# yekaizhou/duet

Measured on AMD Instinct MI355X. Metric: SV support-read marks clustered+phased /sec; bit-exact phased_sv.vcf vs ref, higher is better.
Workload: dtype u32/u64 integer + f64 threshold compares; 1 GPU; BASELINE configs[1]: synthetic 1 contig, 1001116 SV marks / 100000 candidates / 159991 tagged reads, resident in HBM; step = ef_classify + ef_finalize_own, two launches (phasing, E/F; ef_seed_sort 0: ; marks_per_gpu=1001116, candidates_per_gpu=100000, reads_per_gpu=159991, parallelism=contig-sharded x1, svlen_thres=50, suppread_thres=2, device_preheat_steps=2900

## Files before the change

### duet_amd/csrc/duet_ef.hip

```cpp

#include <hip/hip_runtime.h>
#include <hip/hip_ext.h>
#include <stdint.h>
#include <stdio.h>
#include <stdlib.h>
#include <string.h>
#include <string>
#include <vector>

#include "duet_ef.h"
#include "duet_internal.h"

#pragma clang fp contract(off)

namespace {

#ifdef DUET_STAMPS
#define STAMP(k, i) do { if (threadIdx.x == 0 && p.stamps) p.stamps[((size_t)(k) * 65536 + blockIdx.x) * 8 + (i)] = wall_clock64(); } while (0)
#else
#define STAMP(k, i) do { } while (0)
#endif

#include "duet_seeds.hip.h"

// ... 361 lines not shown
                v.t1 = st.TA1; v.t2 = st.TA2;
                bool need_fp = false;
                int pred = (p.dbg & DUET_DBG_EF_FP_DECIDE) ? 0 : decide01_int((int)n_ps, v, deg, svread, refread, need_fp);
                need_fp = need_fp || (p.dbg & DUET_DBG_EF_FP_DECIDE) != 0;
                if (need_fp) pred = decide((int)n_ps, v, deg, svread, refread);
                code = (uint8_t)pred;
                ps_out = st.ps_a == kEmpty ? 0u : st.ps_a;
                if (n_ps == 0 || (st.a1 == 0 && st.a2 == 0)) code |= kNeedNearest;
            }
        }
        p.out_pred[c] = code;
        p.out_ps[c] = ps_out;
    }
    return want_seed ? st.seed() : kEmpty;
}

__device__ __forceinline__ void seeds_tile(const Params &p, TileShared &sh, uint32_t tile, uint32_t tid, uint32_t c,
                                           uint32_t is_start, bool owner = true)
{
    const uint32_t seed = owner ? sh.seed[tid] : kEmpty;
    const bool want_seed = seed != kEmpty;
    const uint32_t lane = tid & 63u, wave = tid >> 6;
    const unsigned long long wmask = __ballot(want_seed);
    const unsigned long long smask = __ballot(is_start != 0);
    const unsigned long long upto = lane == 63 ? ~0ull : ((1ull << (lane + 1)) - 1ull);
    if (lane == 0 && owner) {
        if (wmask) {
            const uint32_t li = 63u - (uint32_t)__clzll(wmask);
            sh.wlast[wave] = sh.seed[wave * 64 + li];
            sh.wclean[wave] = (li == 63 || (smask >> (li + 1)) == 0) ? 1u : 0u;
        } else {
            sh.wlast[wave] = kEmpty;
            sh.wclean[wave] = 0;
        }
    }
    __syncthreads();
    bool keep = want_seed;
    if (want_seed) {
        const unsigned long long lower = wmask & (upto >> 1);
        if (lower) {
            const uint32_t pl = 63u - (uint32_t)__clzll(lower);
            const unsigned long long between = smask & upto & ~((1ull << (pl + 1)) - 1ull);
            keep = !(between == 0 && sh.seed[wave * 64 + pl] == seed);
        } else if (wave > 0) {
            keep = !((smask & upto) == 0 && sh.wclean[wave - 1] && sh.wlast[wave - 1] == seed);
        }
    }
    const unsigned long long mask = __ballot(keep);
    if (lane == 0 && owner) sh.wcnt[wave] = (uint32_t)__popcll(mask);
    __syncthreads();
    uint32_t before = 0, total = 0;
#pragma unroll
    for (uint32_t w = 0; w < kCandPerBlock / 64; ++w) {
        before += w < wave ? sh.wcnt[w] : 0u;
        total += sh.wcnt[w];
    }
    if (keep) {
        const uint32_t at = before + (uint32_t)__popcll(mask & (upto >> 1));
        const uint64_t e = ((uint64_t)c << 32) | seed;
        if (at < 7) p.blk_rec[(size_t)tile * 8 + 1 + at] = e;
        if (at >= 3) p.seed_ent[(size_t)tile * kCandPerBlock + at] = e;
    }
    if (tid == 0) p.blk_rec[(size_t)tile * 8] = total;
}

__device__ __forceinline__ void issue_fence()
{
    asm volatile("" ::: "memory");
    __builtin_amdgcn_sched_barrier(0);
}

template <int NT = kCandPerBlock, int IT>
__device__ __forceinline__ void stage_load_marks(const uint32_t *__restrict__ mark_read, uint4 (&r)[IT], uint32_t cs, uint32_t m_end,
                                                 uint32_t tid)
{
#pragma unroll
    for (int it = 0; it < IT; ++it) {
        const uint32_t m = cs + 4u * (tid + it * NT);
        r[it] = *reinterpret_cast<const uint4 *>(mark_read + (m < m_end ? m : cs));
    }
    issue_fence();
}

template <int IT>
__device__ __forceinline__ void stage_gather(const uint64_t *__restrict__ read_tag, const uint64_t *__restrict__ untagged, uint32_t n_reads,
                                             uint64_t (&t)[4 * IT], const uint4 (&r)[IT])
{
#pragma unroll
    for (int it = 0; it < IT; ++it) {
        uint32_t idx[4] = {r[it].x, r[it].y, r[it].z, r[it].w};
        asm volatile("" : "+v"(idx[0]), "+v"(idx[1]), "+v"(idx[2]), "+v"(idx[3])::"memory");
#pragma unroll
        for (int j = 0; j < 4; ++j) {
            const uint64_t *a = idx[j] < n_reads ? read_tag + idx[j] : untagged;
            t[4 * it + j] = *a;
        }
        issue_fence();
    }
}

template <int NT = kCandPerBlock, int IT4>
__device__ __forceinline__ void stage_store(uint64_t *s_tag, const uint64_t (&t)[IT4], uint32_t tid)
{
#pragma unroll
    for (int it = 0; it < IT4 / 4; ++it) {
        const uint32_t i = 4u * (tid + it * NT);
#pragma unroll
        for (int j = 0; j < 4; ++j) s_tag[i + j] = t[4 * it + j];
    }
}

template <bool VEC, bool DYN = false>
__global__ __launch_bounds__(kCandPerBlock, 6) void ef_classify(const Params p)
{
    __shared__ uint64_t s_tag[kChunk];
    __shared__ uint32_t s_span[2];
    __shared__ TileShared sh;

    const uint32_t tid = threadIdx.x;
    STAMP(0, 0);
    const uint32_t C = p.C, n_reads = p.n_reads, svlen_thres = p.svlen_thres, suppread_thres = p.suppread_thres;
    const uint32_t heavy_t = min(p.heavy_t, 255u);
    const uint32_t *__restrict__ const cand_off = p.cand_off, *__restrict__ const mark_read = p.mark_read;
    const uint64_t *__restrict__ const read_tag = p.read_tag, *__restrict__ const untagged = p.untagged;
    const uint32_t *__restrict__ const cand_svlen = p.cand_svlen, *__restrict__ const cand_svread = p.cand_svread;
    const uint32_t *__restrict__ const cand_refread = p.cand_refread;
    const uint8_t *__restrict__ const cand_gt_ok = p.cand_gt_ok, *__restrict__ const ctg_start = p.ctg_start;
    asm volatile("" ::"s"(C), "s"(n_reads), "s"(svlen_thres), "s"(suppread_thres), "s"(heavy_t), "s"(cand_off), "s"(mark_read),
                 "s"(read_tag), "s"(untagged), "s"(cand_svlen), "s"(cand_svread), "s"(cand_refread), "s"(cand_gt_ok), "s"(ctg_start));
    asm volatile("" ::"s"(p.dbg), "s"(p.out_pred), "s"(p.out_ps), "s"(p.blk_rec), "s"(p.seed_ent), "s"(p.c2rec), "s"(p.status),
                 "s"(p.c2_fixed), "s"(p.c2_cap));
    uint32_t n_cands = C;
    for (uint32_t tile = blockIdx.x;; tile += gridDim.x) {
        const uint32_t c0 = tile * kCandPerBlock, c = c0 + tid;
        const uint32_t ic = min(c, C - 1u);
        const uint32_t o0_ld = cand_off[min(c, C)], o1_ld = cand_off[min(c + 1u, C)];
        const uint32_t svlen_ld = cand_svlen[ic], svread_ld = cand_svread[ic], refread_ld = cand_refread[ic], gt_ld = cand_gt_ok[ic];
        uint32_t start_ld = 0, cc0_ld = 0, cc1_ld = 0, mb_ld = 0, me_ld = 0;
        if constexpr (DYN) {
            if (p.cand_contig) {
                cc0_ld = p.cand_contig[ic];
                cc1_ld = p.cand_contig[max(ic, 1u) - 1u];
            }
        } else {
            start_ld = ctg_start[ic];
            mb_ld = cand_off[c0];
            me_ld = cand_off[min(c0 + (uint32_t)kCandPerBlock, C)];
        }
        if constexpr (DYN) {
            uint32_t zero = 0;
            asm volatile("" : "+s"(zero));
            n_cands = p.dyn_c[zero];
            if (c0 >= n_cands) break;
        }
        const uint32_t nc = min((uint32_t)kCandPerBlock, n_cands - c0);
        asm volatile("" ::"v"(o0_ld), "v"(o1_ld), "v"(svlen_ld), "v"(svread_ld), "v"(refread_ld), "v"(gt_ld), "v"(start_ld), "v"(cc0_ld),
                     "v"(cc1_ld));
        if (tid == 0) sh.c2n = 0;
        const bool live = tid < nc;
        const uint32_t svlen = svlen_ld, svread = svread_ld, refread = refread_ld, gt_ok = gt_ld;
        uint32_t is_start = 0;
        if constexpr (DYN) {
            if (p.cand_contig) {
                is_start = (live && (c == 0 || cc0_ld != cc1_ld)) ? 1u : 0u;
            } else if (live) {
                uint32_t k = p.blk_ctg[tile];
                while (c >= p.ctg_off[k + 1]) ++k;
                is_start = c == p.ctg_off[k] ? 1u : 0u;
            }
        } else {
            is_start = live ? start_ld : 0u;
        }
        const bool kept = live && svlen >= svlen_thres && svread >= suppread_thres && gt_ok != 0;
        const bool divzero = kept && ((uint64_t)svread + (uint64_t)refread == 0);
        uint32_t m_begin, m_end;
        if constexpr (DYN) {
            if (tid == 0) s_span[0] = o0_ld;
            if (tid == nc - 1u) s_span[1] = o1_ld;
            lds_barrier();
            m_begin = s_span[0]; m_end = s_span[1];
        } else {
            m_begin = mb_ld; m_end = me_ld;
        }
        m_begin = (uint32_t)__builtin_amdgcn_readfirstlane((int)m_begin);
        m_end = (uint32_t)__builtin_amdgcn_readfirstlane((int)m_end);
        STAMP(0, 1);

        const uint32_t j = tid;
        const bool active = kept && !divzero;
        const uint32_t my_b = live ? o0_ld : 0, my_e = live ? o1_ld : 0;
        CandState st;

        const uint32_t base = VEC ? (m_begin & ~3u) : m_begin;
        for (uint32_t cs = base; cs < m_end; cs += kChunk) {
            if (VEC) {
                uint4 r[kStageIt];
                uint64_t t[4 * kStageIt];
                stage_load_marks(mark_read, r, cs, m_end, tid);
                stage_gather(read_tag, untagged, n_reads, t, r);
                stage_store(s_tag, t, tid);
            } else {
                for (uint32_t i = tid; i < kChunk && cs + i < m_end; i += kCandPerBlock) {
                    const uint32_t r = mark_read[cs + i];
                    s_tag[i] = r < n_reads ? read_tag[r] : kUntagged;
                }
            }
            __syncthreads();
            STAMP(0, 2);
            uint32_t lo = max(my_b, cs);
            const uint32_t hi = min(my_e, cs + (uint32_t)kChunk);
            if (!kept) lo = hi;
            const bool heavy = lo < hi && my_e - my_b > heavy_t;
            unsigned long long hm = __ballot(heavy);
            consume_range(st, s_tag, heavy ? hi : lo, hi, cs);
            while (hm) {
                const uint32_t h = (uint32_t)__builtin_amdgcn_readfirstlane((int)((uint32_t)__ffsll((long long)hm) - 1u));
                hm &= hm - 1ull;
                const uint32_t lo_h = (uint32_t)__builtin_amdgcn_readlane((int)lo, h), hi_h = (uint32_t)__builtin_amdgcn_readlane((int)hi, h);
                consume_heavy(st, s_tag, lo_h, hi_h, cs, tid & 63u, h);
            }
            STAMP(0, 3);
            __syncthreads();
        }
        STAMP(0, 4);
        uint32_t c2_rank;
        const uint32_t seed = decide_store(p, sh, tile, live, c0 + j, active, divzero, st, my_e - my_b, svread, refread, c2_rank);
        sh.seed[j] = seed;
        __syncthreads();
        if (sh.c2n > kC2Quota) {
            if (tid == 0) sh.c2base = atomicAdd(&p.status[1], sh.c2n - kC2Quota);
            __syncthreads();
            if (live && c2_rank != kEmpty && c2_rank >= kC2Quota) {
                const uint32_t at = sh.c2base + (c2_rank - kC2Quota);
                if (at < p.c2_cap - p.c2_fixed) {
                    store_summary(p, p.c2_fixed + at, st);
                    p.out_pred[c0 + j] = kClass2;
                    p.out_ps[c0 + j] = p.c2_fixed + at;
                }
            }
        }
        seeds_tile(p, sh, tile, tid, c0 + tid, is_start);
        STAMP(0, 6);
        if (!DYN) break;
        __syncthreads();
    }
}

constexpr int kSplit = 2;
constexpr int kSplitThreads = kSplit * kCandPerBlock;
constexpr int kSplitChunk = kChunk;
constexpr int kSplitStagers = 384;
constexpr int kSplitStageIt = kSplitChunk / (kSplitStagers * 4);
constexpr uint32_t kSplitMaxTiles = 512;
static_assert(kSplit == 2 || kSplit == 4, "the parts are halves, or halves of halves");
static_assert(kSplitStageIt >= 1 && kSplitStageIt * kSplitStagers * 4 == kSplitChunk, "a pass is whole 16-byte loads");
static_assert(kSplitStagers % 64 == 0 && kSplitStagers <= kSplitThreads, "whole wavefronts stage");

__device__ __forceinline__ void split_bounds(uint32_t b, uint32_t e, uint32_t part, uint32_t &lo, uint32_t &hi)
{
    lo = b; hi = e;
#pragma unroll
    for (uint32_t bit = kSplit >> 1; bit != 0; bit >>= 1) {
        const uint32_t mid = lo + (hi - lo + 1u) / 2u;
        if (part & bit) lo = mid; else hi = mid;
    }
}

__device__ __forceinline__ void fold(CandState &l, const CandState &r)
{
    l.multi = l.multi || r.multi || (l.first_ps != kEmpty && r.first_ps != kEmpty && l.first_ps != r.first_ps);
    l.first_ps = min(l.first_ps, r.first_ps);
    l.nv += r.nv;
    auto take = [&](uint32_t ps, uint32_t n, uint32_t h1, uint32_t h2, uint32_t t1, uint32_t t2) {
        const bool is = ps != kEmpty;
        const bool to_a = is && (l.ps_a == kEmpty || l.ps_a == ps);
        const bool to_b = is && !to_a && (l.ps_b == kEmpty || l.ps_b == ps);
        l.ps_a = to_a ? ps : l.ps_a;
        l.a1 += to_a ? h1 : 0u; l.a2 += to_a ? h2 : 0u;
        l.TA1 += to_a ? t1 : 0u; l.TA2 += to_a ? t2 : 0u;
        l.ps_b = to_b ? ps : l.ps_b;
        l.n_b += to_b ? n : 0u;
        l.b1 += to_b ? h1 : 0u; l.b2 += to_b ? h2 : 0u;
        l.tb1 += to_b ? t1 : 0u; l.tb2 += to_b ? t2 : 0u;
        l.more = l.more || (is && !to_a && !to_b);
    };
    take(r.ps_a, r.nv - r.n_b, r.a1, r.a2, (uint32_t)r.TA1, (uint32_t)r.TA2);
    take(r.ps_b, r.n_b, r.b1, r.b2, r.tb1, r.tb2);
    l.more = l.more || r.more;
    l.n_a = l.more ? (l.ps_a != kEmpty ? 1u : 0u) : l.nv - l.n_b;
}

__device__ __forceinline__ void hand_store(uint4 (*s_hand)[(kSplit - 1) * kCandPerBlock], uint32_t slot, const CandState &st)
{
    s_hand[0][slot] = make_uint4(st.first_ps, st.ps_a, st.ps_b, st.nv | st.n_b << 8 | (st.multi ? 1u << 16 : 0u) | (st.more ? 1u << 17 : 0u));
    s_hand[1][slot] = make_uint4(st.a1 << 24 | (uint32_t)st.TA1, st.a2 << 24 | (uint32_t)st.TA2, st.b1 << 24 | st.tb1, st.b2 << 24 | st.tb2);
}

__device__ __forceinline__ CandState hand_load(const uint4 (*s_hand)[(kSplit - 1) * kCandPerBlock], uint32_t slot)
{
    const uint4 x = s_hand[0][slot], y = s_hand[1][slot];
    CandState st;
    st.first_ps = x.x; st.ps_a = x.y; st.ps_b = x.z;
    st.nv = x.w & 0xFFu; st.n_b = (x.w >> 8) & 0xFFu; st.multi = (x.w >> 16 & 1u) != 0; st.more = (x.w >> 17 & 1u) != 0;
    st.a1 = y.x >> 24; st.a2 = y.y >> 24; st.b1 = y.z >> 24; st.b2 = y.w >> 24;
    st.TA1 = y.x & 0xFFFFFFu; st.TA2 = y.y & 0xFFFFFFu; st.tb1 = y.z & 0xFFFFFFu; st.tb2 = y.w & 0xFFFFFFu;
    return st;
}

template <bool VEC>
__global__ __launch_bounds__(kSplitThreads, 6) void ef_classify_split(const Params p)
{
    __shared__ uint64_t s_tag[kSplitChunk];
    __shared__ uint4 s_hand[2][(kSplit - 1) * kCandPerBlock];
    __shared__ TileShared sh;

    const uint32_t tid = threadIdx.x, j = tid % kCandPerBlock, part = tid / kCandPerBlock;
    const bool owner = part == 0;
    STAMP(0, 0);
    const uint32_t C = p.C, n_reads = p.n_reads, svlen_thres = p.svlen_thres, suppread_thres = p.suppread_thres;
    const uint32_t heavy_t = min(p.heavy_t, 255u);
    const uint32_t *__restrict__ const cand_off = p.cand_off, *__restrict__ const mark_read = p.mark_read;
    const uint64_t *__restrict__ const read_tag = p.read_tag, *__restrict__ const untagged = p.untagged;
    const uint32_t *__restrict__ const cand_svlen = p.cand_svlen, *__restrict__ const cand_svread = p.cand_svread;
    const uint32_t *__restrict__ const cand_refread = p.cand_refread;
    const uint8_t *__restrict__ const cand_gt_ok = p.cand_gt_ok, *__restrict__ const ctg_start = p.ctg_start;
    asm volatile("" ::"s"(C), "s"(n_reads), "s"(svlen_thres), "s"(suppread_thres), "s"(heavy_t), "s"(cand_off), "s"(mark_read),
                 "s"(read_tag), "s"(untagged), "s"(cand_svlen), "s"(cand_svread), "s"(cand_refread), "s"(cand_gt_ok), "s"(ctg_start));
    asm volatile("" ::"s"(p.dbg), "s"(p.out_pred), "s"(p.out_ps), "s"(p.blk_rec), "s"(p.seed_ent), "s"(p.c2rec), "s"(p.status),
                 "s"(p.c2_fixed), "s"(p.c2_cap));
    const uint32_t tile = blockIdx.x, c0 = tile * kCandPerBlock, c = c0 + j;
    const uint32_t ic = min(c, C - 1u);
    const uint32_t o0_ld = cand_off[min(c, C)], o1_ld = cand_off[min(c + 1u, C)];
    const uint32_t svlen_ld = cand_svlen[ic], svread_ld = cand_svread[ic], refread_ld = cand_refread[ic], gt_ld = cand_gt_ok[ic];
    const uint32_t start_ld = ctg_start[ic];
    const uint32_t mb_ld = cand_off[c0], me_ld = cand_off[min(c0 + (uint32_t)kCandPerBlock, C)];
    const uint32_t nc = min((uint32_t)kCandPerBlock, C - c0);
    asm volatile("" ::"v"(o0_ld), "v"(o1_ld), "v"(svlen_ld), "v"(svread_ld), "v"(refread_ld), "v"(gt_ld), "v"(start_ld));
    if (tid == 0) sh.c2n = 0;
    const bool live = j < nc;
    const uint32_t svlen = svlen_ld, svread = svread_ld, refread = refread_ld, gt_ok = gt_ld;
    const uint32_t is_start = (owner && live) ? start_ld : 0u;
    const bool kept = live && svlen >= svlen_thres && svread >= suppread_thres && gt_ok != 0;
    const bool divzero = kept && ((uint64_t)svread + (uint64_t)refread == 0);
    const uint32_t m_begin = (uint32_t)__builtin_amdgcn_readfirstlane((int)mb_ld);
    const uint32_t m_end = (uint32_t)__builtin_amdgcn_readfirstlane((int)me_ld);
    STAMP(0, 1);

    const bool active = kept && !divzero;
    const uint32_t my_b = live ? o0_ld : 0, my_e = live ? o1_ld : 0;
    const bool heavy_c = my_e - my_b > heavy_t;
    uint32_t w_b, w_e;
    split_bounds(my_b, my_e, part, w_b, w_e);
    if (heavy_c) { w_b = my_b; w_e = owner ? my_e : my_b; }
    if (!kept) w_e = w_b;
    CandState st;

    const uint32_t base = VEC ? (m_begin & ~3u) : m_begin;
    for (uint32_t cs = base; cs < m_end; cs += kSplitChunk) {
        if (VEC) {
            if (tid < kSplitStagers) {
                uint4 r[kSplitStageIt];
                uint64_t t[4 * kSplitStageIt];
                stage_load_marks<kSplitStagers>(mark_read, r, cs, m_end, tid);
                stage_gather(read_tag, untagged, n_reads, t, r);
                stage_store<kSplitStagers>(s_tag, t, tid);
            }
        } else {
            for (uint32_t i = tid; i < kSplitChunk && cs + i < m_end; i += kSplitThreads) {
                const uint32_t r = mark_read[cs + i];
                s_tag[i] = r < n_reads ? read_tag[r] : kUntagged;
            }
        }
        __syncthreads();
        STAMP(0, 2);
        const uint32_t lo = max(w_b, cs), hi = min(w_e, cs + (uint32_t)kSplitChunk);
        const bool heavy = heavy_c && lo < hi;
        unsigned long long hm = __ballot(heavy);
        consume_range(st, s_tag, heavy ? hi : lo, hi, cs);
        while (hm) {
            const uint32_t h = (uint32_t)__builtin_amdgcn_readfirstlane((int)((uint32_t)__ffsll((long long)hm) - 1u));
            hm &= hm - 1ull;
            const uint32_t lo_h = (uint32_t)__builtin_amdgcn_readlane((int)lo, h), hi_h = (uint32_t)__builtin_amdgcn_readlane((int)hi, h);
            consume_heavy(st, s_tag, lo_h, hi_h, cs, tid & 63u, h);
        }
        STAMP(0, 3);
        if (!owner && cs + (uint32_t)kSplitChunk >= m_end) hand_store(s_hand, tid - kCandPerBlock, st);
        __syncthreads();
    }
    STAMP(0, 4);
    uint32_t c2_rank = kEmpty;
    if (owner) {
        if (base < m_end) {
#pragma unroll
            for (int k = 1; k < kSplit; ++k) fold(st, hand_load(s_hand, (k - 1) * kCandPerBlock + j));
        }
        sh.seed[j] = decide_store(p, sh, tile, live, c, active, divzero, st, my_e - my_b, svread, refread, c2_rank);
    }
    __syncthreads();
    if (sh.c2n > kC2Quota) {
        if (tid == 0) sh.c2base = atomicAdd(&p.status[1], sh.c2n - kC2Quota);
        __syncthreads();
        if (owner && live && c2_rank != kEmpty && c2_rank >= kC2Quota) {
            const uint32_t at = sh.c2base + (c2_rank - kC2Quota);
            if (at < p.c2_cap - p.c2_fixed) {
                store_summary(p, p.c2_fixed + at, st);
                p.out_pred[c] = kClass2;
                p.out_ps[c] = p.c2_fixed + at;
            }
        }
    }
    seeds_tile(p, sh, tile, tid, c, is_start, owner);
    STAMP(0, 6);
}


__device__ void bitonic_sort(uint32_t *a, uint32_t n, uint32_t tid, uint32_t nthreads)
{
    uint32_t lN = 0;
    while ((1u << lN) < n) ++lN;
    const uint32_t pairs = (1u << lN) >> 1;
    for (uint32_t lk = 1; lk <= lN; ++lk) {
        const uint32_t k = 1u << lk, half = k >> 1;
        for (uint32_t i = tid; i < pairs; i += nthreads) {
            const uint32_t base = (i >> (lk - 1)) << lk, off = i & (half - 1);
            const uint32_t x = base + off, y = base + (k - 1 - off);
            if (y < n) {
                const uint32_t ax = a[x], ay = a[y];
                if (ax > ay) { a[x] = ay; a[y] = ax; }
            }
        }
        __syncthreads();
        for (int lj = (int)lk - 2; lj >= 0; --lj) {
            const uint32_t j = 1u << lj;
            for (uint32_t i = tid; i < pairs; i += nthreads) {
                const uint32_t x = ((i >> lj) << (lj + 1)) + (i & (j - 1)), y = x + j;
                if (y < n) {
                    const uint32_t ax = a[x], ay = a[y];
                    if (ax > ay) { a[x] = ay; a[y] = ax; }
                }
            }
            __syncthreads();
        }
    }
}

__device__ bool oddeven_rounds(uint32_t *a, uint32_t n, uint32_t tid, uint32_t nthreads, uint32_t *s_flag, int max_rounds)
{
    for (int r = 0; r < max_rounds; ++r) {
        if (tid == 0) *s_flag = 0;
        __syncthreads();
        for (int par = 0; par < 2; ++par) {
            for (uint32_t i = 2 * tid + par; i + 1 < n; i += 2 * nthreads) {
                const uint32_t x = a[i], y = a[i + 1];
                if (x > y) { a[i] = y; a[i + 1] = x; *s_flag = 1; }
            }
            __syncthreads();
        }
        if (*s_flag == 0) return true;
        __syncthreads();
    }
    return false;
}

__device__ uint32_t block_exscan(uint32_t v, uint32_t tid, uint32_t *s_part , uint32_t nthreads,
                                 uint32_t *total)
{
    const uint32_t lane = tid & 63u, wave = tid >> 6;
    uint32_t x = v;
#pragma unroll
    for (int d = 1; d < 64; d <<= 1) {
// ... 812 lines not shown
                                                 uint32_t me_, const uint32_t *s_tab, Vote *vo, uint32_t *pso)
{
    auto each = [&](auto f) {
        for (uint32_t m0 = mb; m0 < me_; m0 += 8) {
            uint32_t r[8];
            uint64_t t[8];
#pragma unroll
            for (int j = 0; j < 8; ++j) r[j] = tagged_index(n_reads, mark_read[m0 + j < me_ ? m0 + j : mb]);
#pragma unroll
            for (int j = 0; j < 8; ++j) t[j] = read_tag[r[j] == kEmpty ? 0u : r[j]];
#pragma unroll
            for (int j = 0; j < 8; ++j)
                if (m0 + j < me_) f(r[j] == kEmpty ? kUntagged : t[j]);
        }
    };
    auto member = [&](uint32_t key) -> bool {
        uint32_t h = (key * 2654435761u) >> (32u - 11u);
        for (;;) {
            const uint32_t v = s_tab[h];
            if (v == key) return true;
            if (v == kEmpty) return false;
            h = (h + 1u) & (kOwnTab - 1u);
        }
    };
    Vote v = {0, 0, 0, 0, 0, 0};
    uint32_t ps = 0, best = 0, done_ps = kEmpty;
    each([&](uint64_t t) {
        if (t != kUntagged && tag_pc(t) <= kPcMax) ++v.allhap;
    });
    each([&](uint64_t t) {
        if (t == kUntagged || tag_pc(t) > kPcMax) return;
        const uint32_t g = tag_ps(t);
        if (g == done_ps || (g == ps && best)) return;
        if (!member(g)) return;
        uint32_t n = 0, n1 = 0, n2 = 0;
        uint64_t s1 = 0, s2 = 0;
        each([&](uint64_t u) {
            if (u == kUntagged || tag_pc(u) > kPcMax || tag_ps(u) != g) return;
            ++n;
            const uint32_t hap = tag_hap(u), pc = tag_pc(u);
            n1 += hap == 1 ? 1u : 0u; s1 += hap == 1 ? pc : 0u;
            n2 += hap == 2 ? 1u : 0u; s2 += hap == 2 ? pc : 0u;
        });
        done_ps = g;
        if (n > best) {
            best = n; ps = g;
            v.hap1 = n1; v.hap2 = n2; v.t1 = s1; v.t2 = s2;
            v.hap0 = v.allhap - n1 - n2;
        }
    });
    *vo = v;
    *pso = ps;
}

__device__ __forceinline__ bool own_probe(uint32_t *s_tab, uint32_t key, uint32_t h)
{
    for (uint32_t probes = 0; probes < kOwnTab; ++probes) {
        const uint32_t old = atomicCAS(&s_tab[h], kEmpty, key);
        if (old == kEmpty) return true;
        if (old == key) return false;
        h = (h + 1u) & (kOwnTab - 1u);
    }
    return false;
}

constexpr uint32_t kOwnWin = 64;

template <uint32_t T>
__device__ __forceinline__ void finalize_own_tiles(const Params &p)
{
    constexpr uint32_t NT = 256u * T, NW = 4u * T;
    static_assert(kOwnTab % NT == 0 && NT <= 1024u, "the clear and own_sort_set deal the table out evenly");
    __shared__ uint32_t s_tab[kOwnTab];
    __shared__ uint32_t s_key[kOwnKeys];
    __shared__ uint32_t s_one[kOwnKeys];
    __shared__ uint32_t s_win[kOwnWin];
    __shared__ uint32_t s_mm[NW][2];
    __shared__ uint32_t s_red[NW][3];
    __shared__ uint32_t s_part[NW];
    __shared__ uint32_t s_nwin;
    __shared__ __align__(8) uint32_t s_c2[T * kC2Quota * kC2Words];
    const uint32_t tid = threadIdx.x, lane = tid & 63u, wave = tid >> 6;
    STAMP(2, 0);
    if (blockIdx.x == 0 && tid == 0) p.status[1] = 0;
    const uint32_t n_cands = p.C;
    const uint32_t nK = p.n_small;
    auto coff = [&](uint32_t kk) -> uint32_t { return p.ctg_small[kk]; };
    const uint32_t tile = blockIdx.x * T;
    const uint32_t c0 = blockIdx.x * NT, c = c0 + tid;
    const bool live = c < n_cands;
    const uint32_t cl = live ? c : n_cands - 1u;
    const uint32_t last = min(c0 + (NT - 1u), n_cands - 1);
    const uint32_t keys_cap = (p.dbg & DUET_DBG_EF_OWN_SMALLTAB) ? 8u : kOwnKeys;
    const uint32_t win_cap = (p.dbg & DUET_DBG_EF_OWN_SMALLTAB) ? 2u : kOwnWin;
    const TileRecs recs{reinterpret_cast<const ulonglong4 *>(p.blk_rec)};
    constexpr uint32_t kPre = 2;
    static_assert(kPre == 2, "the overflow loop selects between rec[0] and rec[1]");
    ulonglong4 rec[kPre], ext[kPre];
    auto load_recs = [&](uint32_t b_lo, uint32_t b_hi) {
#pragma unroll
        for (uint32_t i = 0; i < kPre; ++i) {
            const uint32_t b = min(b_lo + tid + NT * i, b_hi);
            rec[i] = recs[b];
            ext[i] = recs.second(b);
        }
    };
    const uint32_t code_ld = p.out_pred[cl], ps_ld = p.out_ps[cl], pos_ld = p.cand_pos[cl];
    const uint32_t o0_ld = p.cand_off[cl], o1_ld = p.cand_off[cl + 1u];
    const uint32_t sv_ld = p.cand_svread[cl], rf_ld = p.cand_refread[cl];
    constexpr uint32_t kPairs = T * kC2Quota * kC2Words / 2;
    static_assert(kPairs <= 2u * NT, "two pieces per thread");
    const uint2 *c2src = reinterpret_cast<const uint2 *>(p.c2rec + (size_t)tile * kC2Quota * kC2Words);
    const uint2 a0 = c2src[tid], a1 = c2src[tid + NT < kPairs ? tid + NT : tid];
    uint32_t lo = 0, hi = nK;
    while (hi - lo > 1) {
        const uint32_t mid = (lo + hi) >> 1;
        if (coff(mid) <= c0) lo = mid; else hi = mid;
    }
    uint32_t k_first = lo;
    while (k_first < nK && coff(k_first) == coff(k_first + 1)) ++k_first;
    {
        const uint32_t kf = k_first < nK ? k_first : 0u;
        load_recs(coff(kf) / kCandPerBlock, (coff(kf + 1) - 1) / kCandPerBlock);
    }
    asm volatile("" ::"v"(code_ld), "v"(ps_ld), "v"(pos_ld), "v"(o0_ld), "v"(o1_ld), "v"(sv_ld), "v"(rf_ld), "v"(a0.x), "v"(a0.y),
                 "v"(a1.x), "v"(a1.y));
    STAMP(2, 4);
    {
        uint2 *dst = reinterpret_cast<uint2 *>(s_c2);
        dst[tid] = a0;
        if (tid + NT < kPairs) dst[tid + NT] = a1;
    }
    const uint32_t code = live ? code_ld : 0u, ps_in = live ? ps_ld : 0u, c_pos = live ? pos_ld : 0u;
    const uint32_t c_o0 = live ? o0_ld : 0u, c_o1 = live ? o1_ld : 0u;
    const uint32_t c_svread = live ? sv_ld : 0u, c_refread = live ? rf_ld : 0u;
    for (uint32_t k = lo; k < nK && coff(k) <= last; ++k) {
        const uint32_t c_lo = coff(k), c_hi = coff(k + 1);
        if (c_lo == c_hi) continue;
        const uint32_t b_lo = c_lo / kCandPerBlock, b_hi = (c_hi - 1) / kCandPerBlock;
        if (k != k_first) load_recs(b_lo, b_hi);
        uint32_t t_k = threadIdx.x;
        asm volatile("" : "+v"(t_k));
        const uint32_t tid = t_k, lane = t_k & 63u, wave = t_k >> 6;
#pragma unroll
        for (uint32_t i = 0; i < kOwnTab / NT; ++i) s_tab[tid + NT * i] = kEmpty;
        if (tid == 0) s_nwin = 0;
        const bool mine = live && c >= c_lo && c < c_hi;
        const bool asks = mine && code >= 4u && !(code & kDivZero);
        {
            const uint32_t mn = wave_max_u32(asks ? ~c_pos : 0u), mx = wave_max_u32(asks ? c_pos + 1u : 0u);
            if (lane == 0) { s_mm[wave][0] = mn; s_mm[wave][1] = mx; }
        }
        lds_barrier();
        STAMP(2, 1);
        asm volatile("" ::"v"(rec[0].x), "v"(rec[1].x), "v"(rec[0].y), "v"(rec[1].y), "v"(rec[0].z), "v"(rec[1].z), "v"(rec[0].w),
                     "v"(rec[1].w), "v"(ext[0].x), "v"(ext[1].x), "v"(ext[0].y), "v"(ext[1].y), "v"(ext[0].z), "v"(ext[1].z),
                     "v"(ext[0].w), "v"(ext[1].w));
        STAMP(2, 3);
        uint32_t pmin, pmax;
        {
            uint32_t a0 = max(max(s_mm[0][0], s_mm[1][0]), max(s_mm[2][0], s_mm[3][0]));
            uint32_t a1 = max(max(s_mm[0][1], s_mm[1][1]), max(s_mm[2][1], s_mm[3][1]));
#pragma unroll
            for (uint32_t w = 4; w < NW; w += 4) {
                a0 = max(a0, max(max(s_mm[w][0], s_mm[w + 1][0]), max(s_mm[w + 2][0], s_mm[w + 3][0])));
                a1 = max(a1, max(max(s_mm[w][1], s_mm[w + 1][1]), max(s_mm[w + 2][1], s_mm[w + 3][1])));
            }
            pmin = a1 ? ~a0 : 0u;
            pmax = a1 ? a1 - 1u : 0u;
        }
        uint32_t fresh = 0, leftp = 0, rinv = 0;
        static_assert(kOwnTab == 1u << 11, "the hash takes 11 bits");
        auto slot_of = [](uint32_t key) -> uint32_t { return (key * 2654435761u) >> (32u - 11u); };
        auto count_new = [&](bool nw, uint32_t key) {
            fresh += nw ? 1u : 0u;
            leftp = max(leftp, (nw && key <= pmin) ? key + 1u : 0u);
            rinv = max(rinv, (nw && key >= pmax) ? ~key : 0u);
            if (nw && key > pmin && key < pmax) {
                const uint32_t at = atomicAdd(&s_nwin, 1u);
                if (at < kOwnWin) s_win[at] = key;
            }
        };
        auto insert = [&](uint64_t e) {
            const uint32_t cc = (uint32_t)(e >> 32), key = (uint32_t)e;
            if (cc >= c_lo && cc < c_hi) count_new(own_probe(s_tab, key, slot_of(key)), key);
        };
        uint32_t coll = 0;
        auto group = [&](const uint64_t (&e)[4], uint32_t first, uint32_t n_in, uint32_t cnt, uint32_t bit0) {
            uint32_t key[4], old[4];
            bool ok[4];
#pragma unroll
            for (uint32_t j = 0; j < 4; ++j) {
                const uint32_t cc = (uint32_t)(e[j] >> 32);
                key[j] = (uint32_t)e[j];
                ok[j] = j < n_in && first + j < cnt && cc >= c_lo && cc < c_hi;
                old[j] = kEmpty;
            }
#pragma unroll
            for (uint32_t j = 0; j < 4; ++j)
                if (ok[j]) old[j] = atomicCAS(&s_tab[slot_of(key[j])], kEmpty, key[j]);
#pragma unroll
            for (uint32_t j = 0; j < 4; ++j) {
                coll |= (ok[j] && old[j] != kEmpty && old[j] != key[j]) ? 1u << (bit0 + j) : 0u;
                count_new(ok[j] && old[j] == kEmpty, key[j]);
            }
        };
#pragma unroll
        for (uint32_t i = 0; i < kPre; ++i) {
            const uint32_t cnt = b_lo + tid + NT * i <= b_hi ? (uint32_t)rec[i].x : 0u;
            if (__any(cnt > 0u)) {
                const uint64_t e[4] = {rec[i].y, rec[i].z, rec[i].w, 0ull};
                group(e, 0u, 3u, cnt, 7u * i);
            }
            if (__any(cnt > 3u)) {
                const uint64_t e[4] = {ext[i].x, ext[i].y, ext[i].z, ext[i].w};
                group(e, 3u, 4u, cnt, 7u * i + 3u);
            }
        }
        while (coll) {
            const uint32_t j = (uint32_t)__ffs(coll) - 1u;
            coll &= coll - 1u;
            uint32_t key = 0;
#pragma unroll
            for (uint32_t i = 0; i < kPre; ++i) {
                key = j == 7u * i + 0u ? (uint32_t)rec[i].y : key;
                key = j == 7u * i + 1u ? (uint32_t)rec[i].z : key;
                key = j == 7u * i + 2u ? (uint32_t)rec[i].w : key;
                key = j == 7u * i + 3u ? (uint32_t)ext[i].x : key;
                key = j == 7u * i + 4u ? (uint32_t)ext[i].y : key;
                key = j == 7u * i + 5u ? (uint32_t)ext[i].z : key;
                key = j == 7u * i + 6u ? (uint32_t)ext[i].w : key;
            }
            count_new(own_probe(s_tab, key, (slot_of(key) + 1u) & (kOwnTab - 1u)), key);
        }
        auto overflow = [&](uint32_t b, uint32_t cnt, uint32_t from) {
            constexpr uint32_t kLong = 24;
            if (cnt > from && cnt <= kLong) {
// ... 51 lines not shown
        }
        const uint32_t n_win = s_nwin;
        const bool over = u > keys_cap;
        const bool sorted = !over && n_win > win_cap;
        if (sorted) own_sort_set<NT>(s_tab, s_key, s_one, s_part, u, tid);
        STAMP(2, 5);
        auto nearest = [&](uint32_t pos) -> uint32_t {
            if (sorted) return nearest_seed(s_one, u, pos);
            uint32_t best = 0;
            int64_t bd = -1;
            auto look = [&](uint32_t v) {
                const int64_t d = llabs((int64_t)pos - (int64_t)v);
                if (bd < 0 || d < bd || (d == bd && v > best)) { bd = d; best = v; }
            };
            if (Lp) look(Lp - 1u);
            if (Ri) look(~Ri);
            for (uint32_t i = 0; i < n_win; ++i) look(s_win[i]);
            return best;
        };
        auto member = [&](uint32_t key) -> bool {
            uint32_t h = (key * 2654435761u) >> (32u - 11u);
            for (;;) {
                const uint32_t v = s_tab[h];
                if (v == key) return true;
                if (v == kEmpty) return false;
                h = (h + 1u) & (kOwnTab - 1u);
            }
        };
        if (mine) {
            if (u == 0) {
                if (code != 0) p.out_pred[c] = 0;
                if (ps_in != 0) p.out_ps[c] = 0;
            } else if (code >= 4u) {
                if (code & kDivZero) {
                    atomicOr(&p.status[0], 1u);
                    p.out_pred[c] = 0;
                    p.out_ps[c] = 0;
                } else if (over) {
                    const OwnArgs a = {recs, p.seed_ent, p.read_tag, p.cand_pos, p.cand_off, p.cand_svread, p.cand_refread, p.mark_read, p.c2rec,
                                       p.out_ps, p.status, p.out_pred, c_lo, c_hi, p.n_reads};
                    finalize_candidate_walk(a, c, code, ps_in);
                } else if (code & kClass2Slow) {
                    Vote v;
                    uint32_t ps;
                    own_vote_from_marks(p.mark_read, p.read_tag, p.n_reads, c_o0, c_o1, s_tab, &v, &ps);
                    if (v.hap1 == 0 && v.hap2 == 0) ps = nearest(c_pos);
                    p.out_pred[c] = (uint8_t)decide(2, v, c_o1 - c_o0, c_svread, c_refread);
                    p.out_ps[c] = ps;
                } else if (code & kClass2) {
                    uint32_t w[kC2Words];
                    const uint32_t own0 = tile * kC2Quota;
                    if (ps_in >= own0 && ps_in < own0 + T * kC2Quota) {
#pragma unroll
                        for (int i = 0; i < kC2Words; ++i) w[i] = s_c2[(ps_in - own0) * kC2Words + i];
                    } else {
                        const uint32_t *rec2 = p.c2rec + (size_t)ps_in * kC2Words;
#pragma unroll
                        for (int i = 0; i < kC2Words; ++i) w[i] = rec2[i];
                    }
                    Vote v = {0, 0, 0, 0, 0, 0};
                    uint32_t ps = 0, best = 0;
                    v.allhap = w[0];
                    const uint32_t ng = w[1];
#pragma unroll
                    for (int g = 0; g < kC2Groups; ++g) {
                        if ((uint32_t)g < ng && w[2 + 6 * g + 1] > best && member(w[2 + 6 * g])) {
                            best = w[2 + 6 * g + 1];
                            ps = w[2 + 6 * g];
                            v.hap1 = w[2 + 6 * g + 2]; v.hap2 = w[2 + 6 * g + 3];
                            v.t1 = w[2 + 6 * g + 4]; v.t2 = w[2 + 6 * g + 5];
                            v.hap0 = v.allhap - v.hap1 - v.hap2;
                        }
                    }
                    if (v.hap1 == 0 && v.hap2 == 0) ps = nearest(c_pos);
                    p.out_pred[c] = (uint8_t)decide(2, v, c_o1 - c_o0, c_svread, c_refread);
                    p.out_ps[c] = ps;
                } else {
                    p.out_pred[c] = (uint8_t)(code & 3u);
                    p.out_ps[c] = nearest(c_pos);
                }
            }
        }
        STAMP(2, 6);
        __syncthreads();
    }
}

__global__ __launch_bounds__(256) void ef_finalize_own(const Params p) { finalize_own_tiles<1>(p); }

__global__ __launch_bounds__(512) void ef_finalize_own_wide(const Params p) { finalize_own_tiles<2>(p); }

__global__ void plan_mark_starts(const uint32_t *ctg_off, uint32_t K, uint8_t *ctg_start)
{
    const uint32_t k = blockIdx.x * blockDim.x + threadIdx.x;
    if (k < K && ctg_off[k] < ctg_off[k + 1]) ctg_start[ctg_off[k]] = 1;
}


}

thread_local std::string duet_g_last_error;

namespace {

inline int fail(duet_ctx *ctx, int code, const std::string &msg) { return duet_fail(ctx, code, msg); }
inline int reserve(duet_ctx *ctx, DevBuf &b, size_t bytes) { return duet_reserve(ctx, b, bytes); }

size_t c2_slots(uint32_t B, uint32_t C) { return (size_t)B * kC2Quota + (C / 8u > 256u ? C / 8u : 256u); }

struct WsWant { DevBuf *buf[6]; size_t bytes[6]; };
WsWant ws_want(duet_ctx *ctx, uint32_t K, uint32_t C, uint32_t B)
{
    const size_t small_words = (size_t)(K + 1) + K + 8 + (size_t)B + 16 + (size_t)B * 16;
    return WsWant{{&ctx->ws_small, &ctx->ws_start, &ctx->ws_ent, &ctx->ws_one, &ctx->ws_tmp, &ctx->ws_c2},
                  {small_words * 4, C, (size_t)B * kCandPerBlock * 8, ((size_t)C + K + 1) * 4, ((size_t)C + K + 1) * 4, c2_slots(B, C) * kC2Words * 4}};
}
int ws_reserve(duet_ctx *ctx, const WsWant &w, bool &grow)
{
    for (int i = 0; i < 6; ++i) grow = grow || w.bytes[i] > w.buf[i]->cap;
    if (!grow) return DUET_OK;
    HIP_TRY(ctx, hipDeviceSynchronize());
    int rc;
    for (int i = 0; i < 6; ++i)
        if ((rc = reserve(ctx, *w.buf[i], w.bytes[i]))) return rc;
    return DUET_OK;
}
void carve_small(duet_ctx *ctx, uint32_t K, uint32_t B)
{
    uint32_t *w = (uint32_t *)ctx->ws_small.ptr;
    ctx->d_ctg_off = w;            w += K + 1;
    ctx->d_n_one = w;              w += K;
    ctx->d_status = w;             w += 8;
    ctx->d_blk_ctg = w;            w += B;
    w += ((uintptr_t)w & 63) ? (64 - ((uintptr_t)w & 63)) / 4 : 0;
    ctx->d_blk_cnt = w;
}

int ensure_plan(duet_ctx *ctx, const duet_ef_problem *pr, hipStream_t stream)
{
    const uint32_t K = pr->n_contigs, C = pr->n_cands;
    if (ctx->plan_C == C && ctx->plan_off.size() == (size_t)K + 1 && ctx->plan_stream == stream &&
        memcmp(ctx->plan_off.data(), pr->cand_ctg_off, sizeof(uint32_t) * (K + 1)) == 0)
        return DUET_OK;
    const uint32_t B = (C + kCandPerBlock - 1) / kCandPerBlock;
    const WsWant want = ws_want(ctx, K, C, B);
    const size_t stage_bytes = ((size_t)K + 1 + B) * 4;
    bool grow = ctx->plan_stream != stream || stage_bytes > ctx->plan_stage_cap;
    int rc;
    if ((rc = ws_reserve(ctx, want, grow))) return rc;
    if (grow) {
        if (stage_bytes > ctx->plan_stage_cap) {
            if (ctx->plan_stage) HIP_TRY(ctx, hipHostFree(ctx->plan_stage));
            ctx->plan_stage = nullptr;
            ctx->plan_stage_cap = 0;
            HIP_TRY(ctx, hipHostMalloc((void **)&ctx->plan_stage, stage_bytes + stage_bytes / 4 + 4096, hipHostMallocDefault));
            ctx->plan_stage_cap = stage_bytes + stage_bytes / 4 + 4096;
        }
    } else {
        HIP_TRY(ctx, hipEventSynchronize(ctx->plan_ev));
    }
    carve_small(ctx, K, B);
    uint32_t *h_off = ctx->plan_stage, *h_blk = ctx->plan_stage + (K + 1);
    memcpy(h_off, pr->cand_ctg_off, sizeof(uint32_t) * (K + 1));
    {
        uint32_t k = 0;
        for (uint32_t b = 0; b < B; ++b) {
            const uint32_t c = b * kCandPerBlock;
// ... 447 lines not shown
```

Before: 66.94 billion marks/s.

## Issue first mark-read loads early and prefetch next chunk in classify loops

In ef_classify (non-DYN path), the first chunk's mark_read loads are now issued right after the span is known, before the per-candidate setup work, and the chunk loop body moves into a classify_pass helper. In the split classify kernel, the next chunk's mark loads are issued at the end of each iteration so they overlap the barrier and loop overhead. finalize_own_tiles is restructured so the next contig's records load after the current one finishes, and several values are recomputed inside the loop under asm barriers, likely to reduce live registers. The aim is to hide global-load latency and cut register pressure, at the cost of more complex control flow and possibly more VGPRs held across the consume phase.

```diff
diff --git a/duet_amd/csrc/duet_ef.hip b/duet_amd/csrc/duet_ef.hip
--- a/duet_amd/csrc/duet_ef.hip
+++ b/duet_amd/csrc/duet_ef.hip
@@ -467,6 +467,14 @@
     issue_fence();
 }
 
+__device__ __forceinline__ uint32_t stage_load_first(const uint32_t *__restrict__ mark_read, uint32_t cs, uint32_t m_end, uint32_t tid)
+{
+    const uint32_t m = cs + tid;
+    const uint32_t r = mark_read[m < m_end ? m : cs];
+    issue_fence();
+    return r;
+}
+
 template <int IT>
 __device__ __forceinline__ void stage_gather(const uint64_t *__restrict__ read_tag, const uint64_t *__restrict__ untagged, uint32_t n_reads,
                                              uint64_t (&t)[4 * IT], const uint4 (&r)[IT])
@@ -493,6 +501,49 @@
 #pragma unroll
         for (int j = 0; j < 4; ++j) s_tag[i + j] = t[4 * it + j];
     }
+}
+
+template <bool VEC, bool ISSUED>
+__device__ __forceinline__ void classify_pass(const Params &p, uint64_t *s_tag, CandState &st, uint4 (&r)[kStageIt], uint32_t r0,
+                                              const uint32_t *__restrict__ mark_read, const uint64_t *__restrict__ read_tag,
+                                              const uint64_t *__restrict__ untagged, uint32_t n_reads, uint32_t cs, uint32_t m_end,
+                                              uint32_t tid, uint32_t my_b, uint32_t my_e, bool kept, uint32_t heavy_t)
+{
+    if (VEC) {
+        uint64_t t[4 * kStageIt];
+        if constexpr (!ISSUED) {
+            stage_load_marks(mark_read, r, cs, m_end, tid);
+            STAMP(0, 7);
+        }
+        stage_gather(read_tag, untagged, n_reads, t, r);
+        stage_store(s_tag, t, tid);
+    } else {
+        uint32_t i = tid;
+        if constexpr (ISSUED) {
+            if (cs + i < m_end) s_tag[i] = r0 < n_reads ? read_tag[r0] : kUntagged;
+            i += kCandPerBlock;
+        }
+        for (; i < kChunk && cs + i < m_end; i += kCandPerBlock) {
+            const uint32_t rr = mark_read[cs + i];
+            s_tag[i] = rr < n_reads ? read_tag[rr] : kUntagged;
+        }
+    }
+    __syncthreads();
+    STAMP(0, 2);
+    uint32_t lo = max(my_b, cs);
+    const uint32_t hi = min(my_e, cs + (uint32_t)kChunk);
+    if (!kept) lo = hi;
+    const bool heavy = lo < hi && my_e - my_b > heavy_t;
+    unsigned long long hm = __ballot(heavy);
+    consume_range(st, s_tag, heavy ? hi : lo, hi, cs);
+    while (hm) {
+        const uint32_t h = (uint32_t)__builtin_amdgcn_readfirstlane((int)((uint32_t)__ffsll((long long)hm) - 1u));
+        hm &= hm - 1ull;
+        const uint32_t lo_h = (uint32_t)__builtin_amdgcn_readlane((int)lo, h), hi_h = (uint32_t)__builtin_amdgcn_readlane((int)hi, h);
+        consume_heavy(st, s_tag, lo_h, hi_h, cs, tid & 63u, h);
+    }
+    STAMP(0, 3);
+    __syncthreads();
 }
 
 template <bool VEC, bool DYN = false>
@@ -541,9 +592,33 @@
         const uint32_t nc = min((uint32_t)kCandPerBlock, n_cands - c0);
         asm volatile("" ::"v"(o0_ld), "v"(o1_ld), "v"(svlen_ld), "v"(svread_ld), "v"(refread_ld), "v"(gt_ld), "v"(start_ld), "v"(cc0_ld),
                      "v"(cc1_ld));
-        if (tid == 0) sh.c2n = 0;
+        const uint32_t svlen = svlen_ld, svread = svread_ld, refread = refread_ld, gt_ok = gt_ld;
+        CandState st;
+        uint32_t m_begin = 0, m_end = 0;
+        bool has_pass = false;
+        if constexpr (!DYN) {
+            m_begin = (uint32_t)__builtin_amdgcn_readfirstlane((int)mb_ld);
+            m_end = (uint32_t)__builtin_amdgcn_readfirstlane((int)me_ld);
+            STAMP(0, 1);
+            const uint32_t base = VEC ? (m_begin & ~3u) : m_begin;
+            has_pass = base < m_end;
+            if (has_pass) {
+                uint4 r[kStageIt];
+                uint32_t r0 = 0;
+                if constexpr (VEC) stage_load_marks(mark_read, r, base, m_end, tid);
+                else r0 = stage_load_first(mark_read, base, m_end, tid);
+                STAMP(0, 7);
+                const bool live_w = tid < nc;
+                const bool kept_w = live_w && svlen >= svlen_thres && svread >= suppread_thres && gt_ok != 0;
+                const uint32_t b_w = live_w ? o0_ld : 0, e_w = live_w ? o1_ld : 0;
+                if (tid == 0) sh.c2n = 0;
+                classify_pass<VEC, true>(p, s_tag, st, r, r0, mark_read, read_tag, untagged, n_reads, base, m_end, tid, b_w, e_w, kept_w, heavy_t);
+                for (uint32_t cs = base + (uint32_t)kChunk; cs < m_end; cs += kChunk)
+                    classify_pass<VEC, false>(p, s_tag, st, r, r0, mark_read, read_tag, untagged, n_reads, cs, m_end, tid, b_w, e_w, kept_w, heavy_t);
+            }
+        }
+        if (tid == 0 && !has_pass) sh.c2n = 0;
         const bool live = tid < nc;
-        const uint32_t svlen = svlen_ld, svread = svread_ld, refread = refread_ld, gt_ok = gt_ld;
         uint32_t is_start = 0;
         if constexpr (DYN) {
             if (p.cand_contig) {
@@ -558,54 +633,52 @@
         }
         const bool kept = live && svlen >= svlen_thres && svread >= suppread_thres && gt_ok != 0;
         const bool divzero = kept && ((uint64_t)svread + (uint64_t)refread == 0);
-        uint32_t m_begin, m_end;
         if constexpr (DYN) {
             if (tid == 0) s_span[0] = o0_ld;
             if (tid == nc - 1u) s_span[1] = o1_ld;
             lds_barrier();
-            m_begin = s_span[0]; m_end = s_span[1];
-        } else {
-            m_begin = mb_ld; m_end = me_ld;
-        }
-        m_begin = (uint32_t)__builtin_amdgcn_readfirstlane((int)m_begin);
-        m_end = (uint32_t)__builtin_amdgcn_readfirstlane((int)m_end);
-        STAMP(0, 1);
+            m_begin = (uint32_t)__builtin_amdgcn_readfirstlane((int)s_span[0]);
+            m_end = (uint32_t)__builtin_amdgcn_readfirstlane((int)s_span[1]);
+            STAMP(0, 1);
+        }
 
         const uint32_t j = tid;
         const bool active = kept && !divzero;
         const uint32_t my_b = live ? o0_ld : 0, my_e = live ? o1_ld : 0;
-        CandState st;
-
-        const uint32_t base = VEC ? (m_begin & ~3u) : m_begin;
-        for (uint32_t cs = base; cs < m_end; cs += kChunk) {
-            if (VEC) {
-                uint4 r[kStageIt];
-                uint64_t t[4 * kStageIt];
-                stage_load_marks(mark_read, r, cs, m_end, tid);
-                stage_gather(read_tag, untagged, n_reads, t, r);
-                stage_store(s_tag, t, tid);
-            } else {
-                for (uint32_t i = tid; i < kChunk && cs + i < m_end; i += kCandPerBlock) {
-                    const uint32_t r = mark_read[cs + i];
-                    s_tag[i] = r < n_reads ? read_tag[r] : kUntagged;
+
+        if constexpr (DYN) {
+            const uint32_t base = VEC ? (m_begin & ~3u) : m_begin;
+            for (uint32_t cs = base; cs < m_end; cs += kChunk) {
+                if (VEC) {
+                    uint4 r[kStageIt];
+                    uint64_t t[4 * kStageIt];
+                    stage_load_marks(mark_read, r, cs, m_end, tid);
+                    STAMP(0, 7);
+                    stage_gather(read_tag, untagged, n_reads, t, r);
+                    stage_store(s_tag, t, tid);
+                } else {
+                    for (uint32_t i = tid; i < kChunk && cs + i < m_end; i += kCandPerBlock) {
+                        const uint32_t r = mark_read[cs + i];
+                        s_tag[i] = r < n_reads ? read_tag[r] : kUntagged;
+                    }
                 }
-            }
-            __syncthreads();
-            STAMP(0, 2);
-            uint32_t lo = max(my_b, cs);
-            const uint32_t hi = min(my_e, cs + (uint32_t)kChunk);
-            if (!kept) lo = hi;
-            const bool heavy = lo < hi && my_e - my_b > heavy_t;
-            unsigned long long hm = __ballot(heavy);
-            consume_range(st, s_tag, heavy ? hi : lo, hi, cs);
-            while (hm) {
-                const uint32_t h = (uint32_t)__builtin_amdgcn_readfirstlane((int)((uint32_t)__ffsll((long long)hm) - 1u));
-                hm &= hm - 1ull;
-                const uint32_t lo_h = (uint32_t)__builtin_amdgcn_readlane((int)lo, h), hi_h = (uint32_t)__builtin_amdgcn_readlane((int)hi, h);
-                consume_heavy(st, s_tag, lo_h, hi_h, cs, tid & 63u, h);
-            }
-            STAMP(0, 3);
-            __syncthreads();
+                __syncthreads();
+                STAMP(0, 2);
+                uint32_t lo = max(my_b, cs);
+                const uint32_t hi = min(my_e, cs + (uint32_t)kChunk);
+                if (!kept) lo = hi;
+                const bool heavy = lo < hi && my_e - my_b > heavy_t;
+                unsigned long long hm = __ballot(heavy);
+                consume_range(st, s_tag, heavy ? hi : lo, hi, cs);
+                while (hm) {
+                    const uint32_t h = (uint32_t)__builtin_amdgcn_readfirstlane((int)((uint32_t)__ffsll((long long)hm) - 1u));
+                    hm &= hm - 1ull;
+                    const uint32_t lo_h = (uint32_t)__builtin_amdgcn_readlane((int)lo, h), hi_h = (uint32_t)__builtin_amdgcn_readlane((int)hi, h);
+                    consume_heavy(st, s_tag, lo_h, hi_h, cs, tid & 63u, h);
+                }
+                STAMP(0, 3);
+                __syncthreads();
+            }
         }
         STAMP(0, 4);
         uint32_t c2_rank;
@@ -721,15 +794,25 @@
     const uint32_t mb_ld = cand_off[c0], me_ld = cand_off[min(c0 + (uint32_t)kCandPerBlock, C)];
     const uint32_t nc = min((uint32_t)kCandPerBlock, C - c0);
     asm volatile("" ::"v"(o0_ld), "v"(o1_ld), "v"(svlen_ld), "v"(svread_ld), "v"(refread_ld), "v"(gt_ld), "v"(start_ld));
+    const uint32_t m_begin = (uint32_t)__builtin_amdgcn_readfirstlane((int)mb_ld);
+    const uint32_t m_end = (uint32_t)__builtin_amdgcn_readfirstlane((int)me_ld);
+    STAMP(0, 1);
+    const uint32_t base = VEC ? (m_begin & ~3u) : m_begin;
+    const bool stager = tid < kSplitStagers;
+    uint4 r[kSplitStageIt];
+    uint32_t r0 = 0;
+    if (VEC) {
+        if (base < m_end && stager) stage_load_marks<kSplitStagers>(mark_read, r, base, m_end, tid);
+    } else {
+        if (base < m_end) r0 = stage_load_first(mark_read, base, m_end, tid);
+    }
+    STAMP(0, 7);
     if (tid == 0) sh.c2n = 0;
     const bool live = j < nc;
     const uint32_t svlen = svlen_ld, svread = svread_ld, refread = refread_ld, gt_ok = gt_ld;
     const uint32_t is_start = (owner && live) ? start_ld : 0u;
     const bool kept = live && svlen >= svlen_thres && svread >= suppread_thres && gt_ok != 0;
     const bool divzero = kept && ((uint64_t)svread + (uint64_t)refread == 0);
-    const uint32_t m_begin = (uint32_t)__builtin_amdgcn_readfirstlane((int)mb_ld);
-    const uint32_t m_end = (uint32_t)__builtin_amdgcn_readfirstlane((int)me_ld);
-    STAMP(0, 1);
 
     const bool active = kept && !divzero;
     const uint32_t my_b = live ? o0_ld : 0, my_e = live ? o1_ld : 0;
@@ -740,18 +823,16 @@
     if (!kept) w_e = w_b;
     CandState st;
 
-    const uint32_t base = VEC ? (m_begin & ~3u) : m_begin;
-    for (uint32_t cs = base; cs < m_end; cs += kSplitChunk) {
+    for (uint32_t cs = base; cs < m_end;) {
         if (VEC) {
-            if (tid < kSplitStagers) {
-                uint4 r[kSplitStageIt];
+            if (stager) {
                 uint64_t t[4 * kSplitStageIt];
-                stage_load_marks<kSplitStagers>(mark_read, r, cs, m_end, tid);
                 stage_gather(read_tag, untagged, n_reads, t, r);
                 stage_store<kSplitStagers>(s_tag, t, tid);
             }
         } else {
-            for (uint32_t i = tid; i < kSplitChunk && cs + i < m_end; i += kSplitThreads) {
+            if (cs + tid < m_end) s_tag[tid] = r0 < n_reads ? read_tag[r0] : kUntagged;
+            for (uint32_t i = tid + kSplitThreads; i < kSplitChunk && cs + i < m_end; i += kSplitThreads) {
                 const uint32_t r = mark_read[cs + i];
                 s_tag[i] = r < n_reads ? read_tag[r] : kUntagged;
             }
@@ -771,6 +852,14 @@
         STAMP(0, 3);
         if (!owner && cs + (uint32_t)kSplitChunk >= m_end) hand_store(s_hand, tid - kCandPerBlock, st);
         __syncthreads();
+        cs += kSplitChunk;
+        if (cs < m_end) {
+            if (VEC) {
+                if (stager) stage_load_marks<kSplitStagers>(mark_read, r, cs, m_end, tid);
+            } else {
+                r0 = stage_load_first(mark_read, cs, m_end, tid);
+            }
+        }
     }
     STAMP(0, 4);
     uint32_t c2_rank = kEmpty;
@@ -1749,17 +1838,17 @@
     __shared__ __align__(8) uint32_t s_c2[T * kC2Quota * kC2Words];
     const uint32_t tid = threadIdx.x, lane = tid & 63u, wave = tid >> 6;
     STAMP(2, 0);
+    uint32_t dbg = p.dbg;
+    asm volatile("" ::"s"(dbg), "s"(p.n_reads), "s"(p.mark_read), "s"(p.read_tag), "s"(p.seed_ent));
     if (blockIdx.x == 0 && tid == 0) p.status[1] = 0;
     const uint32_t n_cands = p.C;
     const uint32_t nK = p.n_small;
     auto coff = [&](uint32_t kk) -> uint32_t { return p.ctg_small[kk]; };
-    const uint32_t tile = blockIdx.x * T;
-    const uint32_t c0 = blockIdx.x * NT, c = c0 + tid;
+    uint32_t tile = blockIdx.x * T;
+    const uint32_t c0 = blockIdx.x * NT;
+    uint32_t c = c0 + tid;
     const bool live = c < n_cands;
     const uint32_t cl = live ? c : n_cands - 1u;
-    const uint32_t last = min(c0 + (NT - 1u), n_cands - 1);
-    const uint32_t keys_cap = (p.dbg & DUET_DBG_EF_OWN_SMALLTAB) ? 8u : kOwnKeys;
-    const uint32_t win_cap = (p.dbg & DUET_DBG_EF_OWN_SMALLTAB) ? 2u : kOwnWin;
     const TileRecs recs{reinterpret_cast<const ulonglong4 *>(p.blk_rec)};
     constexpr uint32_t kPre = 2;
     static_assert(kPre == 2, "the overflow loop selects between rec[0] and rec[1]");
@@ -1784,12 +1873,11 @@
         const uint32_t mid = (lo + hi) >> 1;
         if (coff(mid) <= c0) lo = mid; else hi = mid;
     }
-    uint32_t k_first = lo;
-    while (k_first < nK && coff(k_first) == coff(k_first + 1)) ++k_first;
-    {
-        const uint32_t kf = k_first < nK ? k_first : 0u;
-        load_recs(coff(kf) / kCandPerBlock, (coff(kf + 1) - 1) / kCandPerBlock);
-    }
+    uint32_t k = lo;
+    while (k < nK && coff(k) == coff(k + 1)) ++k;
+    if (k >= nK) return;
+    uint32_t c_lo = coff(k), c_hi = coff(k + 1);
+    load_recs(c_lo / kCandPerBlock, (c_hi - 1) / kCandPerBlock);
     asm volatile("" ::"v"(code_ld), "v"(ps_ld), "v"(pos_ld), "v"(o0_ld), "v"(o1_ld), "v"(sv_ld), "v"(rf_ld), "v"(a0.x), "v"(a0.y),
                  "v"(a1.x), "v"(a1.y));
     STAMP(2, 4);
@@ -1798,28 +1886,30 @@
         dst[tid] = a0;
         if (tid + NT < kPairs) dst[tid + NT] = a1;
     }
-    const uint32_t code = live ? code_ld : 0u, ps_in = live ? ps_ld : 0u, c_pos = live ? pos_ld : 0u;
-    const uint32_t c_o0 = live ? o0_ld : 0u, c_o1 = live ? o1_ld : 0u;
-    const uint32_t c_svread = live ? sv_ld : 0u, c_refread = live ? rf_ld : 0u;
-    for (uint32_t k = lo; k < nK && coff(k) <= last; ++k) {
-        const uint32_t c_lo = coff(k), c_hi = coff(k + 1);
-        if (c_lo == c_hi) continue;
+    uint32_t code = live ? code_ld : 0u, ps_in = live ? ps_ld : 0u, c_pos = live ? pos_ld : 0u;
+    uint32_t c_o0 = live ? o0_ld : 0u, c_o1 = live ? o1_ld : 0u;
+    uint32_t c_svread = live ? sv_ld : 0u, c_refread = live ? rf_ld : 0u;
+    for (;;) {
         const uint32_t b_lo = c_lo / kCandPerBlock, b_hi = (c_hi - 1) / kCandPerBlock;
-        if (k != k_first) load_recs(b_lo, b_hi);
         uint32_t t_k = threadIdx.x;
         asm volatile("" : "+v"(t_k));
         const uint32_t tid = t_k, lane = t_k & 63u, wave = t_k >> 6;
 #pragma unroll
         for (uint32_t i = 0; i < kOwnTab / NT; ++i) s_tab[tid + NT * i] = kEmpty;
         if (tid == 0) s_nwin = 0;
-        const bool mine = live && c >= c_lo && c < c_hi;
-        const bool asks = mine && code >= 4u && !(code & kDivZero);
         {
+            const bool asks = c >= c_lo && c < c_hi && code >= 4u && !(code & kDivZero);
             const uint32_t mn = wave_max_u32(asks ? ~c_pos : 0u), mx = wave_max_u32(asks ? c_pos + 1u : 0u);
             if (lane == 0) { s_mm[wave][0] = mn; s_mm[wave][1] = mx; }
         }
         lds_barrier();
         STAMP(2, 1);
+        asm volatile("" : "+v"(c), "+v"(code), "+v"(ps_in), "+v"(c_pos), "+v"(c_o0), "+v"(c_o1), "+v"(c_svread), "+v"(c_refread), "+s"(dbg),
+                     "+s"(tile));
+        const bool mine = c >= c_lo && c < c_hi;
+        const uint32_t last = min(tile * kCandPerBlock + (NT - 1u), n_cands - 1u);
+        const uint32_t keys_cap = (dbg & DUET_DBG_EF_OWN_SMALLTAB) ? 8u : kOwnKeys;
+        const uint32_t win_cap = (dbg & DUET_DBG_EF_OWN_SMALLTAB) ? 2u : kOwnWin;
         asm volatile("" ::"v"(rec[0].x), "v"(rec[1].x), "v"(rec[0].y), "v"(rec[1].y), "v"(rec[0].z), "v"(rec[1].z), "v"(rec[0].w),
                      "v"(rec[1].w), "v"(ext[0].x), "v"(ext[1].x), "v"(ext[0].y), "v"(ext[1].y), "v"(ext[0].z), "v"(ext[1].z),
                      "v"(ext[0].w), "v"(ext[1].w));
@@ -2037,7 +2127,13 @@
             }
         }
         STAMP(2, 6);
+        do {
+            if (++k >= nK) return;
+            c_lo = coff(k); c_hi = coff(k + 1);
+        } while (c_lo == c_hi);
+        if (c_lo > last) return;
         __syncthreads();
+        load_recs(c_lo / kCandPerBlock, (c_hi - 1) / kCandPerBlock);
     }
 }
 
```

Measured after the change: 66.32 billion marks/s. Within noise of the previous version (-0.9%).
